# matt-graham/mici

Measured on NVIDIA H100. Metric: leapfrog steps/sec (aggregate over chains), higher is better.
Workload: dtype f64

## Files before the change

mici_b200/csrc/leapfrog_dmma.cuh:

```cuda
#pragma once
#include <type_traits>

#include "targets.cuh"

namespace mb200 {

__device__ __forceinline__ void dmma_m8n8k4(double& c0, double& c1, double a, double b) {
  asm volatile(
      "mma.sync.aligned.m8n8k4.row.col.f64.f64.f64.f64 {%0,%1}, {%2}, {%3}, {%0,%1};\n"
      : "+d"(c0), "+d"(c1)
      : "d"(a), "d"(b));
}

__device__ __forceinline__ void dmma_m16n8k16(double& c0, double& c1, double& c2, double& c3,
                                              const double2 (&a)[2][2], const double2 (&b)[2]) {
  asm volatile(
      "mma.sync.aligned.m16n8k16.row.col.f64.f64.f64.f64 {%0,%1,%2,%3}, "
      "{%4,%5,%6,%7,%8,%9,%10,%11}, {%12,%13,%14,%15}, {%0,%1,%2,%3};\n"
      : "+d"(c0), "+d"(c1), "+d"(c2), "+d"(c3)
      : "d"(a[0][0].x), "d"(a[1][0].x), "d"(a[0][0].y), "d"(a[1][0].y),
        "d"(a[0][1].x), "d"(a[1][1].x), "d"(a[0][1].y), "d"(a[1][1].y),
        "d"(b[0].x), "d"(b[0].y), "d"(b[1].x), "d"(b[1].y));
}

__device__ __forceinline__ uint32_t smem_u32(const void* p) {
  return static_cast<uint32_t>(__cvta_generic_to_shared(p));
}

__device__ __forceinline__ void named_barrier_sync(int id, int nthreads) {
  asm volatile("bar.sync %0, %1;" ::"r"(id), "r"(nthreads) : "memory");
}

#ifndef MB200_K1_TRACE
#define MB200_K1_TRACE(phase)
#endif
#ifndef MB200_K1_TRACE_AFTER
#define MB200_K1_TRACE_AFTER(phase, x)
#endif
#ifndef MB200_K1_MARK
#define MB200_K1_MARK(id)
#endif

constexpr int DMMA_TILES_PER_CTA = 8;
#ifndef MB200_DMMA_GROUPS
#define MB200_DMMA_GROUPS 4
#endif
constexpr int DMMA_GROUPS = MB200_DMMA_GROUPS;
__host__ __device__ constexpr int dmma_tile_count(int g) {
  return DMMA_TILES_PER_CTA / DMMA_GROUPS + (g < DMMA_TILES_PER_CTA % DMMA_GROUPS ? 1 : 0);
}
__host__ __device__ constexpr int dmma_tile_start(int g) {
  return g * (DMMA_TILES_PER_CTA / DMMA_GROUPS) +
         (g < DMMA_TILES_PER_CTA % DMMA_GROUPS ? g : DMMA_TILES_PER_CTA % DMMA_GROUPS);
}
constexpr int DMMA_MAX_MT = (DMMA_TILES_PER_CTA + DMMA_GROUPS - 1) / DMMA_GROUPS;
constexpr int DMMA_THREADS = 32 * 4 * DMMA_GROUPS;
constexpr int DMMA_ROWS_PER_CTA = 8 * DMMA_TILES_PER_CTA;

template <int DP>
struct DmmaSmem {
  static constexpr int LDA = DP + 8;
  double A[DP * LDA];
  double P[DMMA_ROWS_PER_CTA * LDA];
  double psum[DMMA_ROWS_PER_CTA][4];
  double rscal[DMMA_ROWS_PER_CTA];
  double ex[2][DMMA_ROWS_PER_CTA][4];
  unsigned long long mbar;
};

template <class Target, int DP, int MT, bool PC>
__device__ __forceinline__ void leapfrog_dmma_group(
    DmmaSmem<DP>& sm, const Target& target, const double* q_in, const double* p_in,
    double* q_out, double* p_out, const int32_t* __restrict__ dir,
    const double* __restrict__ step_sizes, int64_t n_chains, int dim,
    double step_size, int n_steps, double* __restrict__ h_out, int32_t* __restrict__ status,
    int32_t* __restrict__ n_done, int64_t chain0, int row0, int w, int lane, int bar_id,
    int cta_threads, bool vec2, int32_t* __restrict__ counters) {
  constexpr int LDA = DmmaSmem<DP>::LDA;
  constexpr int NT = DP / 32;
  constexpr int KS = DP / 4;
  const int r = lane >> 2, c = lane & 3;
  const int col0 = w * (DP / 4);
  const double mh = -0.5 * step_size;
  const bool owner = (w == 0) && (c == 0);

  double q[MT][NT][2], mhr[PC ? MT : 1];
  bool live[MT];
  int row[MT];
  auto load_scale = [&](int64_t ch) {
    const double d = (dir != nullptr && dir[ch] < 0) ? -1.0 : 1.0;
    return PC ? d * step_sizes[ch] : d;
  };
  const uint32_t pofs = (uint32_t)((row0 + r) * LDA + col0 + 2 * c);
  auto pslot = [&](int mt, int nt) -> double2& {
    return *reinterpret_cast<double2*>(&sm.P[pofs + mt * 8 * LDA + 8 * nt]);
  };

#pragma unroll
  for (int mt = 0; mt < MT; ++mt) {
    row[mt] = row0 + 8 * mt + r;
    const int64_t ch = chain0 + row[mt];
    live[mt] = ch < n_chains;
    const double sgn = live[mt] ? load_scale(ch) : (PC ? 0.0 : 1.0);
    if (PC) mhr[mt] = -0.5 * (sgn * sgn);
#pragma unroll
    for (int nt = 0; nt < NT; ++nt) {
      const int i = col0 + 8 * nt + 2 * c;
      double2 a = make_double2(0.0, 0.0), b = make_double2(0.0, 0.0);
      if (live[mt] && i < dim) {
        if (vec2) {
          a = *reinterpret_cast<const double2*>(q_in + (size_t)ch * dim + i);
          b = *reinterpret_cast<const double2*>(p_in + (size_t)ch * dim + i);
        } else {
          a.x = q_in[(size_t)ch * dim + i], b.x = p_in[(size_t)ch * dim + i];
          if (i + 1 < dim) a.y = q_in[(size_t)ch * dim + i + 1], b.y = p_in[(size_t)ch * dim + i + 1];
        }
      }
      q[mt][nt][0] = a.x, q[mt][nt][1] = a.y;
      pslot(mt, nt) = make_double2(sgn * b.x, sgn * b.y);
    }
  }

  int s = -1;

  auto tile_sums = [&]() {
    if (!Target::TILE_SUM) return;
    double v[MT];
#pragma unroll
    for (int mt = 0; mt < MT; ++mt) {
      double t0 = q[mt][0][0] * q[mt][0][0];
      if (Target::COORD0) t0 = owner ? 0.0 : t0;
      t0 = fma(q[mt][0][1], q[mt][0][1], t0);
      if (mt == 0) MB200_K1_TRACE_AFTER(6, t0);
      double t1 = 0.0;
#pragma unroll
      for (int nt = 1; nt < NT; ++nt) {
        double& t = (nt & 1) ? t1 : t0;
        t = fma(q[mt][nt][0], q[mt][nt][0], t);
        t = fma(q[mt][nt][1], q[mt][nt][1], t);
      }
      v[mt] = t0 + t1;
    }
#pragma unroll
    for (int mt = 0; mt < MT; ++mt) v[mt] += __shfl_xor_sync(FULL_MASK, v[mt], 1);
#pragma unroll
    for (int mt = 0; mt < MT; ++mt) v[mt] += __shfl_xor_sync(FULL_MASK, v[mt], 2);
#pragma unroll
    for (int mt = 0; mt < MT; ++mt)
      if (c == 0) sm.psum[row[mt]][w] = v[mt];
  };
  auto publish_partials = [&]() {
    if (Target::ROW_SCALAR && w == 0) {
      double v0 = (c == 0) ? q[0][0][0] : 0.0;
#pragma unroll
      for (int mt = 1; mt < MT; ++mt) {
        const double vm = __shfl_sync(FULL_MASK, q[mt][0][0], lane & ~3);
        v0 = (c == mt) ? vm : v0;
      }
      tile_sums();
      const double rs = target.row_scalar(v0);
      if (c < MT) sm.rscal[row0 + 8 * c + r] = rs;
    } else {
      tile_sums();
    }
  };

  auto update_phase = [&](auto kicks_tag) {
    constexpr int KICKS = decltype(kicks_tag)::value;
    double2 pv[MT][NT];
    if (KICKS > 0) {
#pragma unroll
      for (int mt = 0; mt < MT; ++mt)
#pragma unroll
        for (int nt = 0; nt < NT; ++nt) pv[mt][nt] = pslot(mt, nt);
    }
    publish_partials();
    MB200_K1_TRACE(2);
    named_barrier_sync(bar_id, 128);
    MB200_K1_TRACE(3);
    if (KICKS == 0) return;
    double rs[MT];
#pragma unroll
    for (int mt = 0; mt < MT; ++mt) rs[mt] = Target::ROW_SCALAR ? sm.rscal[row[mt]] : 1.0;
#pragma unroll
    for (int mt = 0; mt < MT; ++mt) {
      const double mhm = PC ? mhr[PC ? mt : 0] : mh;
      const double coef = target.kick_coef(mhm, rs[mt]);
      double c00 = coef, a00 = q[mt][0][0];
      if (Target::COORD0 && w == 0) {
        const double4 ps = *reinterpret_cast<const double4*>(&sm.psum[row[mt]][0]);
        const double g0 = target.grad0(q[mt][0][0], ((ps.x + ps.y) + ps.z) + ps.w, rs[mt]);
        c00 = owner ? mhm : coef;
        a00 = owner ? g0 : a00;
      }
#pragma unroll
      for (int nt = 0; nt < NT; ++nt) {
        double2 v = pv[mt][nt];
        if (Target::LINEAR) {
#pragma unroll
          for (int k = 0; k < KICKS; ++k) {
            v.x = (nt == 0) ? fma(c00, a00, v.x) : fma(coef, q[mt][nt][0], v.x);
            v.y = fma(coef, q[mt][nt][1], v.y);
          }
        } else {
#pragma unroll
          for (int k = 0; k < KICKS; ++k)
            target.kick_pair_nl(mhm, q[mt][nt][0], q[mt][nt][1], v.x, v.y);
        }
        pslot(mt, nt) = v;
      }
    }
    MB200_K1_TRACE(4);
    named_barrier_sync(bar_id, 128);
    MB200_K1_TRACE(5);
  };
  using K0 = std::integral_constant<int, 0>;
  using K1 = std::integral_constant<int, 1>;
  using K2 = std::integral_constant<int, 2>;

  auto drift = [&](double (&acc)[MT][NT][2]) {
    const double2* a_base = reinterpret_cast<const double2*>(&sm.P[(row0 + r) * LDA + 2 * c]);
    const double2* b_base = reinterpret_cast<const double2*>(&sm.A[(col0 + r) * LDA + 2 * c]);
    if constexpr (MT == 2) {
#pragma unroll 2
      for (int j = 0; j < KS / 4; ++j) {
        double2 a[2][2], b[NT][2];
#pragma unroll
        for (int mt = 0; mt < 2; ++mt)
#pragma unroll
          for (int h = 0; h < 2; ++h) a[mt][h] = a_base[mt * 4 * LDA + 4 * (2 * j + h)];
#pragma unroll
        for (int nt = 0; nt < NT; ++nt)
#pragma unroll
          for (int h = 0; h < 2; ++h) b[nt][h] = b_base[nt * 4 * LDA + 4 * (2 * j + h)];
#pragma unroll
        for (int nt = 0; nt < NT; ++nt)
          dmma_m16n8k16(acc[0][nt][0], acc[0][nt][1], acc[1][nt][0], acc[1][nt][1], a, b[nt]);
      }
    } else {
      constexpr bool KSPLIT = (MT == 1);
      double acc2[KSPLIT ? NT : 1][2];
      if (KSPLIT) {
#pragma unroll
        for (int nt = 0; nt < NT; ++nt) acc2[nt][0] = 0.0, acc2[nt][1] = 0.0;
      }
#pragma unroll 4
      for (int j = 0; j < KS / 2; ++j) {
        double2 a[MT], b[NT];
#pragma unroll
        for (int mt = 0; mt < MT; ++mt) a[mt] = a_base[mt * 4 * LDA + 4 * j];
#pragma unroll
        for (int nt = 0; nt < NT; ++nt) b[nt] = b_base[nt * 4 * LDA + 4 * j];
#pragma unroll
        for (int mt = 0; mt < MT; ++mt)
#pragma unroll
          for (int nt = 0; nt < NT; ++nt)
            dmma_m8n8k4(acc[mt][nt][0], acc[mt][nt][1], a[mt].x, b[nt].x);
#pragma unroll
        for (int mt = 0; mt < MT; ++mt)
#pragma unroll
          for (int nt = 0; nt < NT; ++nt) {
            if (KSPLIT) dmma_m8n8k4(acc2[nt][0], acc2[nt][1], a[mt].y, b[nt].y);
            else dmma_m8n8k4(acc[mt][nt][0], acc[mt][nt][1], a[mt].y, b[nt].y);
          }
      }
      if (KSPLIT) {
#pragma unroll
        for (int nt = 0; nt < NT; ++nt) acc[0][nt][0] += acc2[nt][0], acc[0][nt][1] += acc2[nt][1];
      }
    }
  };

  MB200_K1_MARK(4);
  if (n_steps > 0) update_phase(K1{});
  else update_phase(K0{});
  MB200_K1_MARK(5);
  for (s = 0; s < n_steps - 1; ++s) {
    MB200_K1_TRACE(0);
    drift(q);
    MB200_K1_TRACE(1);
    update_phase(K2{});
  }
  if (n_steps > 0) {
    drift(q);
    update_phase(K1{});
  }

  MB200_K1_MARK(6);
#pragma unroll
  for (int mt = 0; mt < MT; ++mt) {
    const int64_t ch = chain0 + row[mt];
    if (!live[mt]) continue;
    const double sgn = load_scale(ch);
#pragma unroll
    for (int nt = 0; nt < NT; ++nt) {
      const int i = col0 + 8 * nt + 2 * c;
      if (i < dim) {
        const double2 sv = pslot(mt, nt);
        double2 pv = make_double2(sgn * sv.x, sgn * sv.y);
        if (PC) {
          if (sgn != 0.0) {
            pv = make_double2(sv.x / sgn, sv.y / sgn);
          } else {
            pv.x = p_in[(size_t)ch * dim + i];
            pv.y = (i + 1 < dim) ? p_in[(size_t)ch * dim + i + 1] : 0.0;
          }
        }
        if (vec2) {
          *reinterpret_cast<double2*>(q_out + (size_t)ch * dim + i) =
              make_double2(q[mt][nt][0], q[mt][nt][1]);
          *reinterpret_cast<double2*>(p_out + (size_t)ch * dim + i) = pv;
        } else {
          q_out[(size_t)ch * dim + i] = q[mt][nt][0], p_out[(size_t)ch * dim + i] = pv.x;
          if (i + 1 < dim)
            q_out[(size_t)ch * dim + i + 1] = q[mt][nt][1], p_out[(size_t)ch * dim + i + 1] = pv.y;
        }
      }
    }
    if (w == 0 && c == 0) {
      if (status != nullptr) status[ch] = MB200_STATUS_OK;
      if (n_done != nullptr) n_done[ch] = n_steps;
      if (counters != nullptr) counters[ch * MB200_N_COUNTERS + MB200_COUNT_GRAD] += n_steps + 1;
    }
  }

  MB200_K1_MARK(7);
  if (h_out != nullptr) {
    double l[MT], kin[MT], u[MT][NT][2];
#pragma unroll
    for (int mt = 0; mt < MT; ++mt) {
      double red[2] = {0.0, 1.0};
      if (Target::TILE_SUM) {
        const double4 ps = *reinterpret_cast<const double4*>(&sm.psum[row[mt]][0]);
        red[0] = ((ps.x + ps.y) + ps.z) + ps.w;
      }
      if (Target::ROW_SCALAR) red[1] = sm.rscal[row[mt]];
      l[mt] = 0.0;
#pragma unroll
      for (int nt = 0; nt < NT; ++nt) {
        const int i = col0 + 8 * nt + 2 * c;
        if (i < dim) l[mt] += target.nld_pair(i, q[mt][nt][0], q[mt][nt][1], red);
        u[mt][nt][0] = 0.0, u[mt][nt][1] = 0.0;
      }
    }
    drift(u);
#pragma unroll
    for (int mt = 0; mt < MT; ++mt) {
      kin[mt] = 0.0;
#pragma unroll
      for (int nt = 0; nt < NT; ++nt) {
        const double2 sv = pslot(mt, nt);
        kin[mt] = fma(sv.x, u[mt][nt][0], kin[mt]);
        kin[mt] = fma(sv.y, u[mt][nt][1], kin[mt]);
      }
      kin[mt] += __shfl_xor_sync(FULL_MASK, kin[mt], 1);
      kin[mt] += __shfl_xor_sync(FULL_MASK, kin[mt], 2);
      l[mt] += __shfl_xor_sync(FULL_MASK, l[mt], 1);
      l[mt] += __shfl_xor_sync(FULL_MASK, l[mt], 2);
      if (c == 0) {
        sm.ex[0][row[mt]][w] = kin[mt];
        sm.ex[1][row[mt]][w] = l[mt];
      }
    }
    named_barrier_sync(bar_id, 128);
    if (w == 0 && c == 0) {
#pragma unroll
      for (int mt = 0; mt < MT; ++mt) {
        if (!live[mt]) continue;
        const double4 k4 = *reinterpret_cast<const double4*>(&sm.ex[0][row[mt]][0]);
        const double4 l4 = *reinterpret_cast<const double4*>(&sm.ex[1][row[mt]][0]);
        const double ks = ((k4.x + k4.y) + k4.z) + k4.w;
        const double ls = ((l4.x + l4.y) + l4.z) + l4.w;
        if (PC) {
          const double e = step_sizes[chain0 + row[mt]];
          h_out[chain0 + row[mt]] = ls + 0.5 * (ks / (e * e));
        } else {
          h_out[chain0 + row[mt]] = ls + 0.5 * (ks / step_size);
        }
      }
    }
  }
}

template <class Target, int DP, bool PC>
__global__ void __launch_bounds__(DMMA_THREADS, 1)
    leapfrog_dmma_kernel(const double* q_in, const double* p_in, double* q_out, double* p_out,
                         const int32_t* __restrict__ dir, const double* __restrict__ step_sizes,
                         int64_t n_chains, int dim,
                         double step_size, int n_steps, const double* __restrict__ minv,
                         ModelArgs model, double* __restrict__ h_out,
                         int32_t* __restrict__ status, int32_t* __restrict__ n_done,
                         int tiles_per_cta, int vec2, int tma_rows) {
  extern __shared__ __align__(128) unsigned char smem_raw[];
  DmmaSmem<DP>& sm = *reinterpret_cast<DmmaSmem<DP>*>(smem_raw);
  constexpr int LDA = DmmaSmem<DP>::LDA;
  const int tid = threadIdx.x;
  const int lane = tid & 31;
  const int warp = tid >> 5;
  const int group = warp >> 2;
  const int w = ((warp & 3) + group) & 3;
  const Target target(model, dim);
  MB200_K1_MARK(0);

  const uint32_t mbar = smem_u32(&sm.mbar);
  if (tma_rows && warp == 0) {
    if (lane == 0) {
      asm volatile("mbarrier.init.shared::cta.b64 [%0], 1;" ::"r"(mbar));
      asm volatile("fence.mbarrier_init.release.cluster;" ::: "memory");
    }
    __syncwarp();
    const uint32_t row_bytes = (uint32_t)dim * 8u;
    if (lane == 0)
      asm volatile("mbarrier.arrive.expect_tx.shared::cta.b64 _, [%0], %1;" ::"r"(mbar),
                   "r"(row_bytes * (uint32_t)dim)
                   : "memory");
    __syncwarp();
#pragma unroll 1
    for (int row = lane; row < dim; row += 32) {
      const unsigned long long src =
          reinterpret_cast<unsigned long long>(minv) + (unsigned long long)row * row_bytes;
      asm volatile(
          "cp.async.bulk.shared::cluster.global.mbarrier::complete_tx::bytes [%0], [%1], %2, [%3];"
          ::"r"(smem_u32(&sm.A[row * LDA])),
          "l"(src), "r"(row_bytes), "r"(mbar)
          : "memory");
    }
  }
  {
    const int64_t chain0 = (int64_t)blockIdx.x * (8 * tiles_per_cta);
    const int64_t left = n_chains - chain0;
    const int64_t rows = left < 8 * tiles_per_cta ? left : 8 * tiles_per_cta;
    const int64_t lines = (rows * dim * 8 + 127) / 128;
    for (int64_t i = tid; i < 2 * lines; i += blockDim.x) {
      const double* base = (i < lines ? q_in : p_in) + (size_t)chain0 * dim;
      const char* ptr = reinterpret_cast<const char*>(base) + (i < lines ? i : i - lines) * 128;
      asm volatile("prefetch.global.L2 [%0];" ::"l"(ptr));
    }
  }
  if (!tma_rows) {
    for (int idx = tid; idx < dim * dim; idx += blockDim.x) {
      const int row = idx / dim, col = idx - row * dim;
      sm.A[row * LDA + col] = minv[idx];
    }
  }
  if (dim < DP) {
    for (int idx = tid; idx < DP * DP; idx += blockDim.x) {
      const int row = idx / DP, col = idx - row * DP;
      if (row >= dim || col >= dim) sm.A[row * LDA + col] = 0.0;
    }
  }
  MB200_K1_MARK(1);
  __syncthreads();
  if (tma_rows) {
    uint32_t done = 0;
    while (!done) {
      asm volatile(
          "{\n .reg .pred p;\n mbarrier.try_wait.parity.shared::cta.b64 p, [%1], 0;\n"
          " selp.u32 %0, 1, 0, p;\n}"
          : "=r"(done)
          : "r"(mbar)
          : "memory");
    }
  }
  MB200_K1_MARK(2);
  if (!PC)
#pragma unroll 4
  for (int idx = tid; idx < DP * (DP / 2); idx += blockDim.x) {
    const int row = idx / (DP / 2), c2 = idx - row * (DP / 2);
    double2* ptr = reinterpret_cast<double2*>(&sm.A[row * LDA]) + c2;
    double2 v = *ptr;
    v.x *= step_size, v.y *= step_size;
    *ptr = v;
  }
  __syncthreads();
  MB200_K1_MARK(3);

  const int rows_per_cta = 8 * tiles_per_cta;
  for (int64_t blk = blockIdx.x; blk * rows_per_cta < n_chains; blk += gridDim.x) {
    const int64_t chain0 = blk * rows_per_cta;
    const int64_t left = n_chains - chain0;
    const int tiles = (int)((left >= rows_per_cta) ? tiles_per_cta : (left + 7) / 8);
    const int base = tiles / DMMA_GROUPS, rem = tiles % DMMA_GROUPS;
    const int mt = base + (group < rem ? 1 : 0);
    const int row0 = 8 * (group * base + (group < rem ? group : rem));
    const int cta_threads = 128 * (tiles < DMMA_GROUPS ? tiles : DMMA_GROUPS);
#define MB200_GROUP(MT)                                                                       \
  leapfrog_dmma_group<Target, DP, MT, PC>(sm, target, q_in, p_in, q_out, p_out, dir,          \
                                          step_sizes, n_chains, dim, step_size, n_steps,      \
                                          h_out, status, n_done, chain0, row0, w, lane,       \
                                          1 + group, cta_threads, vec2 != 0, model.counters)
    if (DMMA_MAX_MT >= 4 && mt == 4) MB200_GROUP(4);
    else if (DMMA_MAX_MT >= 3 && mt == 3) MB200_GROUP(3);
    else if (mt == 2) MB200_GROUP(2);
    else if (mt == 1) MB200_GROUP(1);
#undef MB200_GROUP
    __syncthreads();
  }
}

template <class Target, int DP, bool PC>
static int launch_dmma(const double* q_in, const double* p_in, double* q_out, double* p_out,
                       const int32_t* dir, const double* step_sizes, int64_t n, int dim,
                       double eps, int n_steps,
                       const double* minv, const ModelArgs& m, double* h_out, int32_t* status,
                       int32_t* n_done, cudaStream_t st, int sms) {
  auto kern = leapfrog_dmma_kernel<Target, DP, PC>;
  const size_t smem = sizeof(DmmaSmem<DP>);
  if (cudaFuncSetAttribute(kern, cudaFuncAttributeMaxDynamicSharedMemorySize, (int)smem) !=
      cudaSuccess)
    return MB200_ERR_CUDA;
  const int64_t total_tiles = (n + 7) / 8;
  int64_t tpc = (total_tiles + sms - 1) / sms;
  if (tpc > DMMA_TILES_PER_CTA) tpc = DMMA_TILES_PER_CTA;
  int64_t blocks = (total_tiles + tpc - 1) / tpc;
  if (blocks > sms) blocks = sms;
  auto al16 = [](const void* ptr) { return (reinterpret_cast<uintptr_t>(ptr) & 15) == 0; };
  const int even = (dim & 1) == 0;
  const int vec2 = even && al16(q_in) && al16(p_in) && al16(q_out) && al16(p_out);
  const int tma_rows = even && al16(minv);
  kern<<<(unsigned)blocks, DMMA_THREADS, smem, st>>>(q_in, p_in, q_out, p_out, dir, step_sizes, n,
                                                     dim, PC ? 1.0 : eps, n_steps, minv, m, h_out,
                                                     status, n_done, (int)tpc, vec2, tma_rows);
  return 0;
}

template <class Target>
static int dispatch_dmma_dim(const double* q_in, const double* p_in, double* q_out, double* p_out,
                             const int32_t* dir, const double* step_sizes, int64_t n, int dim,
                             double eps, int n_steps,
                             const double* minv, const ModelArgs& m, double* h_out,
                             int32_t* status, int32_t* n_done, cudaStream_t st, int sms) {
#define MB200_DM(DP)                                                                        \
  return step_sizes != nullptr                                                              \
             ? launch_dmma<Target, DP, true>(q_in, p_in, q_out, p_out, dir, step_sizes, n,  \
                                             dim, eps, n_steps, minv, m, h_out, status,     \
                                             n_done, st, sms)                               \
             : launch_dmma<Target, DP, false>(q_in, p_in, q_out, p_out, dir, nullptr, n,    \
                                              dim, eps, n_steps, minv, m, h_out, status,    \
                                              n_done, st, sms)
  if (dim <= 32) MB200_DM(32);
  if (dim <= 64) MB200_DM(64);
  if (dim <= 96) MB200_DM(96);
  MB200_DM(128);
#undef MB200_DM
}

int leapfrog_dmma_dispatch(const double* q_in, const double* p_in, double* q_out, double* p_out,
                           const int32_t* dir, const double* step_sizes, int64_t n, int dim,
                           double eps, int n_steps,
                           const double* minv, const ModelArgs& m, double* h_out, int32_t* status,
                           int32_t* n_done, cudaStream_t st) {
  if (dim > 128 || dim < 8) return MB200_ERR_UNSUPPORTED;
  if (step_sizes == nullptr && (!(eps != 0.0) || !isfinite(eps)))
    return MB200_ERR_UNSUPPORTED;
  int dev = 0, sms = 132;
  cudaGetDevice(&dev);
  cudaDeviceGetAttribute(&sms, cudaDevAttrMultiProcessorCount, dev);
#define MB200_ARGS                                                                             \
  q_in, p_in, q_out, p_out, dir, step_sizes, n, dim, eps, n_steps, minv, m, h_out, status, n_done, \
      st, sms
  switch (m.target_id) {
    case MB200_TARGET_STD_GAUSSIAN: return dispatch_dmma_dim<StdGaussianTarget>(MB200_ARGS);
    case MB200_TARGET_NEAL_FUNNEL: return dispatch_dmma_dim<NealFunnelTarget>(MB200_ARGS);
    case MB200_TARGET_BANANA: return dispatch_dmma_dim<BananaTarget>(MB200_ARGS);
    default: return MB200_ERR_UNSUPPORTED;
  }
#undef MB200_ARGS
}

}
```

Before: 1.386 billion.

## Overlap metric matrix staging with chain state loads via mbarriers

Moves the wait for the TMA load of the metric matrix and its step-size scaling to after each group has issued its global loads of q and p, so the state loads overlap with staging the matrix. A second mbarrier, counted per warp, replaces the CTA-wide __syncthreads after scaling, and TMA row issue is spread across all warps instead of only warp 0. The explicit L2 prefetch of chain state is dropped. This adds register pressure from holding the raw p values, and relies on every warp reaching the staging callback, including groups with no tiles.

```diff
diff --git a/mici_b200/csrc/leapfrog_dmma.cuh b/mici_b200/csrc/leapfrog_dmma.cuh
--- a/mici_b200/csrc/leapfrog_dmma.cuh
+++ b/mici_b200/csrc/leapfrog_dmma.cuh
@@ -31,6 +31,18 @@
   asm volatile("bar.sync %0, %1;" ::"r"(id), "r"(nthreads) : "memory");
 }
 
+__device__ __forceinline__ void mbar_wait(uint32_t bar, uint32_t parity) {
+  uint32_t done = 0;
+  while (!done) {
+    asm volatile(
+        "{\n .reg .pred p;\n mbarrier.try_wait.parity.shared::cta.b64 p, [%1], %2;\n"
+        " selp.u32 %0, 1, 0, p;\n}"
+        : "=r"(done)
+        : "r"(bar), "r"(parity)
+        : "memory");
+  }
+}
+
 #ifndef MB200_K1_TRACE
 #define MB200_K1_TRACE(phase)
 #endif
@@ -66,16 +78,18 @@
   double rscal[DMMA_ROWS_PER_CTA];
   double ex[2][DMMA_ROWS_PER_CTA][4];
   unsigned long long mbar;
+  unsigned long long mbar_a;
 };
 
-template <class Target, int DP, int MT, bool PC>
+template <class Target, int DP, int MT, bool PC, class StageMetric>
 __device__ __forceinline__ void leapfrog_dmma_group(
     DmmaSmem<DP>& sm, const Target& target, const double* q_in, const double* p_in,
     double* q_out, double* p_out, const int32_t* __restrict__ dir,
     const double* __restrict__ step_sizes, int64_t n_chains, int dim,
     double step_size, int n_steps, double* __restrict__ h_out, int32_t* __restrict__ status,
     int32_t* __restrict__ n_done, int64_t chain0, int row0, int w, int lane, int bar_id,
-    int cta_threads, bool vec2, int32_t* __restrict__ counters) {
+    int cta_threads, bool vec2, int32_t* __restrict__ counters,
+    const StageMetric& stage_metric, bool first) {
   constexpr int LDA = DmmaSmem<DP>::LDA;
   constexpr int NT = DP / 32;
   constexpr int KS = DP / 4;
@@ -96,13 +110,15 @@
     return *reinterpret_cast<double2*>(&sm.P[pofs + mt * 8 * LDA + 8 * nt]);
   };
 
+  double2 p0[MT][NT];
+  double sgn[MT];
 #pragma unroll
   for (int mt = 0; mt < MT; ++mt) {
     row[mt] = row0 + 8 * mt + r;
     const int64_t ch = chain0 + row[mt];
     live[mt] = ch < n_chains;
-    const double sgn = live[mt] ? load_scale(ch) : (PC ? 0.0 : 1.0);
-    if (PC) mhr[mt] = -0.5 * (sgn * sgn);
+    sgn[mt] = live[mt] ? load_scale(ch) : (PC ? 0.0 : 1.0);
+    if (PC) mhr[mt] = -0.5 * (sgn[mt] * sgn[mt]);
 #pragma unroll
     for (int nt = 0; nt < NT; ++nt) {
       const int i = col0 + 8 * nt + 2 * c;
@@ -117,9 +133,15 @@
         }
       }
       q[mt][nt][0] = a.x, q[mt][nt][1] = a.y;
-      pslot(mt, nt) = make_double2(sgn * b.x, sgn * b.y);
-    }
-  }
+      p0[mt][nt] = b;
+    }
+  }
+  if (first) stage_metric();
+#pragma unroll
+  for (int mt = 0; mt < MT; ++mt)
+#pragma unroll
+    for (int nt = 0; nt < NT; ++nt)
+      pslot(mt, nt) = make_double2(sgn[mt] * p0[mt][nt].x, sgn[mt] * p0[mt][nt].y);
 
   int s = -1;
 
@@ -380,6 +402,7 @@
       }
     }
   }
+  MB200_K1_MARK(8);
 }
 
 template <class Target, int DP, bool PC>
@@ -402,21 +425,34 @@
   const Target target(model, dim);
   MB200_K1_MARK(0);
 
-  const uint32_t mbar = smem_u32(&sm.mbar);
-  if (tma_rows && warp == 0) {
-    if (lane == 0) {
-      asm volatile("mbarrier.init.shared::cta.b64 [%0], 1;" ::"r"(mbar));
-      asm volatile("fence.mbarrier_init.release.cluster;" ::: "memory");
-    }
-    __syncwarp();
-    const uint32_t row_bytes = (uint32_t)dim * 8u;
-    if (lane == 0)
+  const uint32_t mbar = smem_u32(&sm.mbar), mbar_a = smem_u32(&sm.mbar_a);
+  const uint32_t row_bytes = (uint32_t)dim * 8u;
+  if (tid == 0) {
+    if (tma_rows) asm volatile("mbarrier.init.shared::cta.b64 [%0], 1;" ::"r"(mbar));
+    asm volatile("mbarrier.init.shared::cta.b64 [%0], %1;" ::"r"(mbar_a), "r"(DMMA_THREADS / 32));
+    asm volatile("fence.mbarrier_init.release.cluster;" ::: "memory");
+    if (tma_rows)
       asm volatile("mbarrier.arrive.expect_tx.shared::cta.b64 _, [%0], %1;" ::"r"(mbar),
                    "r"(row_bytes * (uint32_t)dim)
                    : "memory");
-    __syncwarp();
-#pragma unroll 1
-    for (int row = lane; row < dim; row += 32) {
+  }
+  if (!tma_rows) {
+    for (int idx = tid; idx < dim * dim; idx += blockDim.x) {
+      const int row = idx / dim, col = idx - row * dim;
+      sm.A[row * LDA + col] = minv[idx];
+    }
+  }
+  if (dim < DP) {
+    for (int idx = tid; idx < DP * DP; idx += blockDim.x) {
+      const int row = idx / DP, col = idx - row * DP;
+      if (row >= dim || col >= dim) sm.A[row * LDA + col] = 0.0;
+    }
+  }
+  MB200_K1_MARK(1);
+  __syncthreads();
+  if (tma_rows) {
+    const int row = warp + (DMMA_THREADS / 32) * lane;
+    if (row < dim) {
       const unsigned long long src =
           reinterpret_cast<unsigned long long>(minv) + (unsigned long long)row * row_bytes;
       asm volatile(
@@ -426,54 +462,23 @@
           : "memory");
     }
   }
-  {
-    const int64_t chain0 = (int64_t)blockIdx.x * (8 * tiles_per_cta);
-    const int64_t left = n_chains - chain0;
-    const int64_t rows = left < 8 * tiles_per_cta ? left : 8 * tiles_per_cta;
-    const int64_t lines = (rows * dim * 8 + 127) / 128;
-    for (int64_t i = tid; i < 2 * lines; i += blockDim.x) {
-      const double* base = (i < lines ? q_in : p_in) + (size_t)chain0 * dim;
-      const char* ptr = reinterpret_cast<const char*>(base) + (i < lines ? i : i - lines) * 128;
-      asm volatile("prefetch.global.L2 [%0];" ::"l"(ptr));
-    }
-  }
-  if (!tma_rows) {
-    for (int idx = tid; idx < dim * dim; idx += blockDim.x) {
-      const int row = idx / dim, col = idx - row * dim;
-      sm.A[row * LDA + col] = minv[idx];
-    }
-  }
-  if (dim < DP) {
-    for (int idx = tid; idx < DP * DP; idx += blockDim.x) {
-      const int row = idx / DP, col = idx - row * DP;
-      if (row >= dim || col >= dim) sm.A[row * LDA + col] = 0.0;
-    }
-  }
-  MB200_K1_MARK(1);
-  __syncthreads();
-  if (tma_rows) {
-    uint32_t done = 0;
-    while (!done) {
-      asm volatile(
-          "{\n .reg .pred p;\n mbarrier.try_wait.parity.shared::cta.b64 p, [%1], 0;\n"
-          " selp.u32 %0, 1, 0, p;\n}"
-          : "=r"(done)
-          : "r"(mbar)
-          : "memory");
-    }
-  }
-  MB200_K1_MARK(2);
-  if (!PC)
+  auto stage_metric = [&]() {
+    if (tma_rows) mbar_wait(mbar, 0);
+    MB200_K1_MARK(2);
+    if (!PC)
 #pragma unroll 4
-  for (int idx = tid; idx < DP * (DP / 2); idx += blockDim.x) {
-    const int row = idx / (DP / 2), c2 = idx - row * (DP / 2);
-    double2* ptr = reinterpret_cast<double2*>(&sm.A[row * LDA]) + c2;
-    double2 v = *ptr;
-    v.x *= step_size, v.y *= step_size;
-    *ptr = v;
-  }
-  __syncthreads();
-  MB200_K1_MARK(3);
+    for (int idx = tid; idx < DP * (DP / 2); idx += blockDim.x) {
+      const int row = idx / (DP / 2), c2 = idx - row * (DP / 2);
+      double2* ptr = reinterpret_cast<double2*>(&sm.A[row * LDA]) + c2;
+      double2 v = *ptr;
+      v.x *= step_size, v.y *= step_size;
+      *ptr = v;
+    }
+    __syncwarp();
+    if (lane == 0) asm volatile("mbarrier.arrive.shared::cta.b64 _, [%0];" ::"r"(mbar_a) : "memory");
+    mbar_wait(mbar_a, 0);
+    MB200_K1_MARK(3);
+  };
 
   const int rows_per_cta = 8 * tiles_per_cta;
   for (int64_t blk = blockIdx.x; blk * rows_per_cta < n_chains; blk += gridDim.x) {
@@ -484,15 +489,18 @@
     const int mt = base + (group < rem ? 1 : 0);
     const int row0 = 8 * (group * base + (group < rem ? group : rem));
     const int cta_threads = 128 * (tiles < DMMA_GROUPS ? tiles : DMMA_GROUPS);
+    const bool first = blk == blockIdx.x;
 #define MB200_GROUP(MT)                                                                       \
   leapfrog_dmma_group<Target, DP, MT, PC>(sm, target, q_in, p_in, q_out, p_out, dir,          \
                                           step_sizes, n_chains, dim, step_size, n_steps,      \
                                           h_out, status, n_done, chain0, row0, w, lane,       \
-                                          1 + group, cta_threads, vec2 != 0, model.counters)
+                                          1 + group, cta_threads, vec2 != 0, model.counters,  \
+                                          stage_metric, first)
     if (DMMA_MAX_MT >= 4 && mt == 4) MB200_GROUP(4);
     else if (DMMA_MAX_MT >= 3 && mt == 3) MB200_GROUP(3);
     else if (mt == 2) MB200_GROUP(2);
     else if (mt == 1) MB200_GROUP(1);
+    else if (first) stage_metric();
 #undef MB200_GROUP
     __syncthreads();
   }
```

New measurement: 1.403 billion, median of 6. 1.2% higher.

## Overlap own-slice drift MMA with kick phase and spread TMA row issue across warps

Applied to the files above, without the earlier changes.

After the post-kick barrier, each warp immediately computes its own k-block of the next drift using the freshly kicked momenta still held in registers. The remaining drift k-blocks are then visited in a rotated order starting after that owned block. This starts tensor-core work earlier and staggers shared-memory access across warps, aiming to cut barrier idle time and bank conflicts. Separately, the initial load of the inverse-mass matrix and the scaling of the input momenta are restructured: bulk-copy row issue is spread over all warps behind a __syncthreads, and input loads are grouped before the scaled stores to shared memory. This adds register pressure and more index arithmetic per drift.

```diff
diff --git a/mici_b200/csrc/leapfrog_dmma.cuh b/mici_b200/csrc/leapfrog_dmma.cuh
--- a/mici_b200/csrc/leapfrog_dmma.cuh
+++ b/mici_b200/csrc/leapfrog_dmma.cuh
@@ -96,13 +96,14 @@
     return *reinterpret_cast<double2*>(&sm.P[pofs + mt * 8 * LDA + 8 * nt]);
   };
 
+  double2 pin[MT][NT];
+  double sgn[MT];
 #pragma unroll
   for (int mt = 0; mt < MT; ++mt) {
     row[mt] = row0 + 8 * mt + r;
     const int64_t ch = chain0 + row[mt];
     live[mt] = ch < n_chains;
-    const double sgn = live[mt] ? load_scale(ch) : (PC ? 0.0 : 1.0);
-    if (PC) mhr[mt] = -0.5 * (sgn * sgn);
+    sgn[mt] = live[mt] ? load_scale(ch) : (PC ? 0.0 : 1.0);
 #pragma unroll
     for (int nt = 0; nt < NT; ++nt) {
       const int i = col0 + 8 * nt + 2 * c;
@@ -117,11 +118,40 @@
         }
       }
       q[mt][nt][0] = a.x, q[mt][nt][1] = a.y;
-      pslot(mt, nt) = make_double2(sgn * b.x, sgn * b.y);
-    }
+      pin[mt][nt] = b;
+    }
+  }
+#pragma unroll
+  for (int mt = 0; mt < MT; ++mt) {
+    if (PC) mhr[mt] = -0.5 * (sgn[mt] * sgn[mt]);
+#pragma unroll
+    for (int nt = 0; nt < NT; ++nt)
+      pslot(mt, nt) = make_double2(sgn[mt] * pin[mt][nt].x, sgn[mt] * pin[mt][nt].y);
   }
 
   int s = -1;
+
+  auto kblock16 = [&](double (&acc)[MT][NT][2], const double2 (&a)[2][2], int J) {
+    if constexpr (MT == 2) {
+      const double2* b_base = reinterpret_cast<const double2*>(&sm.A[(col0 + r) * LDA + 2 * c]);
+      double2 b[NT][2];
+#pragma unroll
+      for (int nt = 0; nt < NT; ++nt)
+#pragma unroll
+        for (int h = 0; h < 2; ++h) b[nt][h] = b_base[nt * 4 * LDA + 4 * (2 * J + h)];
+#pragma unroll
+      for (int nt = 0; nt < NT; ++nt)
+        dmma_m16n8k16(acc[0][nt][0], acc[0][nt][1], acc[1][nt][0], acc[1][nt][1], a, b[nt]);
+    }
+  };
+  constexpr bool ROT = (MT == 2) && (DP == 64 || DP == 128);
+  constexpr int JO = DP / 64;
+  auto drift_own = [&](const double2 (&pv)[MT][NT]) {
+    if constexpr (ROT) {
+      const double2 a[2][2] = {{pv[0][0], pv[0][1]}, {pv[1][0], pv[1][1]}};
+      kblock16(q, a, JO * w);
+    }
+  };
 
   auto tile_sums = [&]() {
     if (!Target::TILE_SUM) return;
@@ -165,7 +195,7 @@
     }
   };
 
-  auto update_phase = [&](auto kicks_tag) {
+  auto update_phase = [&](auto kicks_tag, auto next_drift_tag) {
     constexpr int KICKS = decltype(kicks_tag)::value;
     double2 pv[MT][NT];
     if (KICKS > 0) {
@@ -195,7 +225,7 @@
       }
 #pragma unroll
       for (int nt = 0; nt < NT; ++nt) {
-        double2 v = pv[mt][nt];
+        double2& v = pv[mt][nt];
         if (Target::LINEAR) {
 #pragma unroll
           for (int k = 0; k < KICKS; ++k) {
@@ -213,31 +243,33 @@
     MB200_K1_TRACE(4);
     named_barrier_sync(bar_id, 128);
     MB200_K1_TRACE(5);
+    if (decltype(next_drift_tag)::value) drift_own(pv);
+    MB200_K1_TRACE(7);
   };
   using K0 = std::integral_constant<int, 0>;
   using K1 = std::integral_constant<int, 1>;
   using K2 = std::integral_constant<int, 2>;
-
-  auto drift = [&](double (&acc)[MT][NT][2]) {
+  using Next = std::true_type;
+  using Last = std::false_type;
+  using Rotated = std::true_type;
+  using Full = std::false_type;
+
+  auto drift = [&](double (&acc)[MT][NT][2], auto rotated_tag) {
     const double2* a_base = reinterpret_cast<const double2*>(&sm.P[(row0 + r) * LDA + 2 * c]);
-    const double2* b_base = reinterpret_cast<const double2*>(&sm.A[(col0 + r) * LDA + 2 * c]);
     if constexpr (MT == 2) {
+      constexpr bool R = ROT && decltype(rotated_tag)::value;
 #pragma unroll 2
-      for (int j = 0; j < KS / 4; ++j) {
-        double2 a[2][2], b[NT][2];
+      for (int i = R ? 1 : 0; i < KS / 4; ++i) {
+        const int j = R ? (JO * w + i) & (KS / 4 - 1) : i;
+        double2 a[2][2];
 #pragma unroll
         for (int mt = 0; mt < 2; ++mt)
 #pragma unroll
           for (int h = 0; h < 2; ++h) a[mt][h] = a_base[mt * 4 * LDA + 4 * (2 * j + h)];
-#pragma unroll
-        for (int nt = 0; nt < NT; ++nt)
-#pragma unroll
-          for (int h = 0; h < 2; ++h) b[nt][h] = b_base[nt * 4 * LDA + 4 * (2 * j + h)];
-#pragma unroll
-        for (int nt = 0; nt < NT; ++nt)
-          dmma_m16n8k16(acc[0][nt][0], acc[0][nt][1], acc[1][nt][0], acc[1][nt][1], a, b[nt]);
+        kblock16(acc, a, j);
       }
     } else {
+      const double2* b_base = reinterpret_cast<const double2*>(&sm.A[(col0 + r) * LDA + 2 * c]);
       constexpr bool KSPLIT = (MT == 1);
       double acc2[KSPLIT ? NT : 1][2];
       if (KSPLIT) {
@@ -272,18 +304,18 @@
   };
 
   MB200_K1_MARK(4);
-  if (n_steps > 0) update_phase(K1{});
-  else update_phase(K0{});
+  if (n_steps > 0) update_phase(K1{}, Next{});
+  else update_phase(K0{}, Last{});
   MB200_K1_MARK(5);
   for (s = 0; s < n_steps - 1; ++s) {
     MB200_K1_TRACE(0);
-    drift(q);
+    drift(q, Rotated{});
     MB200_K1_TRACE(1);
-    update_phase(K2{});
+    update_phase(K2{}, Next{});
   }
   if (n_steps > 0) {
-    drift(q);
-    update_phase(K1{});
+    drift(q, Rotated{});
+    update_phase(K1{}, Last{});
   }
 
   MB200_K1_MARK(6);
@@ -343,7 +375,7 @@
         u[mt][nt][0] = 0.0, u[mt][nt][1] = 0.0;
       }
     }
-    drift(u);
+    drift(u, Full{});
 #pragma unroll
     for (int mt = 0; mt < MT; ++mt) {
       kin[mt] = 0.0;
@@ -403,20 +435,19 @@
   MB200_K1_MARK(0);
 
   const uint32_t mbar = smem_u32(&sm.mbar);
-  if (tma_rows && warp == 0) {
-    if (lane == 0) {
+  if (tma_rows) {
+    const uint32_t row_bytes = (uint32_t)dim * 8u;
+    if (tid == 0) {
       asm volatile("mbarrier.init.shared::cta.b64 [%0], 1;" ::"r"(mbar));
       asm volatile("fence.mbarrier_init.release.cluster;" ::: "memory");
-    }
-    __syncwarp();
-    const uint32_t row_bytes = (uint32_t)dim * 8u;
-    if (lane == 0)
       asm volatile("mbarrier.arrive.expect_tx.shared::cta.b64 _, [%0], %1;" ::"r"(mbar),
                    "r"(row_bytes * (uint32_t)dim)
                    : "memory");
-    __syncwarp();
+    }
+    __syncthreads();
+    const int nwarps = DMMA_THREADS / 32;
 #pragma unroll 1
-    for (int row = lane; row < dim; row += 32) {
+    for (int row = warp + nwarps * lane; row < dim; row += 32 * nwarps) {
       const unsigned long long src =
           reinterpret_cast<unsigned long long>(minv) + (unsigned long long)row * row_bytes;
       asm volatile(
```

Measured after the change: 1.449 billion before, 1.492 billion after (median of 6 runs). +2.9%, better.
